# orange-vertex/depthmapX

Hardware: AMD Instinct MI355X
Metric: grid cells/sec for VISPREP makeGraph + VGA global on N×N grid (higher is better)
Workload: dtype f64

## Files before the change

### depthmapx_amd/csrc/api/vga_global.hip

```cpp

static void prep_range(const dmx_graph* g, int64_t& b, int64_t& e) {
    b = 0; e = g->nnodes;
    if (g->prep_fn && g->prep_e >= 0) { b = g->prep_b; e = g->prep_e; }
}
static int prep_allreduce(dmx_graph* g, void* p, int64_t count, int dtype) {
    if (!g->prep_fn || count <= 0) return DMX_OK;
    HIPCHK(hipStreamSynchronize(g->ctx->stream));
    if (g->prep_fn(p, count, dtype, g->prep_user) != 0)
        return fail(DMX_ERR_STATE, "prep all-reduce callback failed");
    return DMX_OK;
}
static int prepare_symmetry(dmx_graph* g);
static int build_scan_order(dmx_graph* g);
static int prepare_uf(dmx_graph* g) {
    if (g->scan_ready) return DMX_OK;
    if (int rc = prepare_symmetry(g)) return rc;
    dmx_ctx* ctx = g->ctx;
    hipStream_t s = ctx->stream;
    PointMapHost& h = *g->pm->host;
    const int cols = h.cols(), rows = h.rows();
    const int tw = (cols + 7) / 8, th = (rows + 7) / 8;
    const int64_t C = (int64_t)cols * rows, N = g->nnodes;
    DevBuf<int> cov;
    DevBuf<unsigned long long> cnt;
// ... 47 lines not shown
    if (N) {
        HIPCHK(hipMemcpyAsync(d_ss.p, ss.data(), N * 8, hipMemcpyHostToDevice, s));
        hipLaunchKernelGGL(scan_pool_kernel, dim3((unsigned)std::min<int64_t>(N, 8192)), dim3(256), 0, s, rows,
                           g->pm->d_node_cell.p, N, g->node_run_start.p, g->node_nruns.p, g->bin_nruns.p, g->pool.p, d_ss.p,
                           g->scan_pool.p, g->cell_scan_start.p, g->cell_nruns.p);
        HIPCHK(hipGetLastError());
    }
    HIPCHK(hipStreamSynchronize(s));
    g->scan_released = false;
    return DMX_OK;
}

static int restore_scan_order(dmx_graph* g) {
    if (!g->scan_released) return DMX_OK;
    g->pmask.reset(); g->ppre.reset(); g->poff.reset();
    g->tvis.reset(); g->ftvis.reset(); g->tvsum.reset(); g->tvnz.reset(); g->ttvis.reset();
    g->tvw = 0;
    g->tiles_ready = false;
    return build_scan_order(g);
}

static int prepare_symmetry(dmx_graph* g) {
    if (g->symmetric >= 0) return DMX_OK;
    const char* force = getenv("DMX_VGA_KERNEL");
    if (force && std::string(force) == "topdown") {
        g->symmetric = 0;
        g->sym_diff.reset(); g->sym_ho.reset(); g->sym_fused = false;
        return DMX_OK;
    }
    dmx_ctx* ctx = g->ctx;
    hipStream_t s = ctx->stream;
// ... 185 lines not shown
    }
    return DMX_OK;
}

static void prep_state_stats(dmx_ctx* ctx, const dmx_graph* g) {
    long long f = 0;
    if (g->scan_pool.p) f |= 1;
    if (g->scan_released) f |= 2;
    if (g->tvis.p) f |= 4;
    if (g->ftvis.p) f |= 8;
    if (g->ttvis.p) f |= 16;
    if (g->pmask.p) f |= 32;
    if (g->tvsum.p || g->tvnz.p) f |= 64;
    ctx->last_stats[40] = f;
    ctx->last_stats[41] = (long long)((g->tvis.p ? g->tvis.n * 8 : 0) + (g->ftvis.p ? g->ftvis.n * 8 : 0) +
                                      (g->ttvis.p ? g->ttvis.n * 8 : 0) + (g->tvsum.p ? g->tvsum.n * 8 : 0) + (g->tvnz.p ? g->tvnz.n * 8 : 0));
    ctx->last_stats[42] = (long long)(g->scan_pool.p ? g->scan_pool.n * sizeof(Run) : 0);
}

static size_t tile_lds_layout(int tw, int th, bool* fg, bool* rbm) {
    const size_t nt = (size_t)tw * th, wr_ = (tw + 63) / 64, wc_ = (th + 63) / 64;
    const size_t lds_f = nt * 8, lds_h = (size_t)VGA_HMAX * 4;
    const size_t lds_sc = (size_t)(th * wr_ + tw * wc_) * 8, lds_rbcb = (size_t)(th * wr_ + th * 8 * wr_ + tw * 8 * wc_) * 8;
    const size_t lds_cap = (size_t)160 * 1024 - 1024;
    const char* rb_env = getenv("DMX_VGA_RB");
    const bool rb_ok = !(rb_env && atoi(rb_env) == 0);
    *fg = false;
    *rbm = false;
    if (rb_ok && lds_f + lds_rbcb + lds_h <= lds_cap) { *rbm = true; return lds_f + lds_rbcb + lds_h; }
    if (lds_f + lds_sc + lds_h <= lds_cap) return lds_f + lds_sc + lds_h;
    if (rb_ok && lds_rbcb + lds_h <= lds_cap) { *fg = true; *rbm = true; return lds_rbcb + lds_h; }
// ... 98 lines not shown
        }
        const char* pm_env = getenv("DMX_VGA_PMASK");
        if (ftv && !(pm_env && atoi(pm_env) == 0) && (!wide || ((tvw + 63) / 64 <= 64 && nt <= 65535)))
            if (int rc = prepare_pmask(g, rows, tw, th, tvw, Ct, wide)) return rc;
        if (wide && (tvw + 63) / 64 <= 64) {
            HIPCHK(g->tvsum.alloc((size_t)Ct * ((tvw + 63) / 64)));
            hipLaunchKernelGGL(tile_vsum_kernel, dim3((unsigned)((Ct + 3) / 4)), dim3(256), 0, s, Ct, tvw, g->tvis.p,
                               g->tvsum.p);
            HIPCHK(hipGetLastError());
        }
        const char* nz_env = getenv("DMX_VGA_TVNZ");
        if (VGA_TVNZ && !wide && ftv && g->pmask.p && !(nz_env && atoi(nz_env) == 0)) {
            HIPCHK(g->tvnz.alloc((size_t)Ct * ((tvw + 63) / 64)));
            hipLaunchKernelGGL(tile_vsum_kernel, dim3((unsigned)((Ct + 3) / 4)), dim3(256), 0, s, Ct, tvw, g->tvis.p,
                               g->tvnz.p);
            HIPCHK(hipGetLastError());
        }
        g->tvw = tvw;
    }
    HIPCHK(hipStreamSynchronize(s));
    g->tiles_ready = true;
    return DMX_OK;
}

#ifndef VGA_NT_BIG
#define VGA_NT_BIG 1024
#endif
static int ordered_search(dmx_ctx* ctx, dmx_graph* g, double radius, const std::vector<int32_t>& src,
                          const std::vector<int32_t>& seed_cells, float* outp, int64_t* d_levels, int32_t* d_cell_level) {
    const PointMapHost& h = *g->pm->host;
// ... 74 lines not shown
    return rc;
}

extern "C++" template <int NT, bool SPECIAL, bool RBM, bool FG>
static int launch_tile(dmx_ctx* ctx, const VgaTileParams& Q, int64_t nsrc, size_t lds, int64_t* blocks_out,
                       DevBuf<unsigned long long>& xg, DevBuf<int4>& queue, DevBuf<int32_t>& list) {
    {
        const int64_t nt = (int64_t)Q.tw * Q.th;
        const char* why = nullptr;
        if (Q.tw != (Q.cols + 7) / 8 || Q.th != (Q.rows + 7) / 8 || nt <= 0) why = "tile grid does not cover the cells";
        else if (lds > (size_t)160 * 1024) why = "dynamic LDS above 160 KiB";
        else if (!FG && (size_t)nt * 8 > lds) why = "frontier bitmap larger than the dynamic LDS";
        else if (Q.tvis && Q.tvw != Q.th * ((Q.tw + 63) / 64)) why = "tile-visibility row width differs from the tile grid";
        else if (!FG && Q.pmask && Q.tvw > 256) why = "row words past the fused phase-C test (256)";
        else if (Q.tvnz && (FG || Q.tvw > 256)) why = "narrow row summaries on a wide grid";
        else if (Q.pmask && !FG && nt > 32767) why = "narrow mask hint: tile index above 15 bits";
        else if (Q.asym_tiles && Q.alist_cap <= 0) why = "asymmetric mode without an A-cell list";
        if (why) return fail(DMX_ERR_STATE, (std::string("VGA tile launch: ") + why).c_str());
        hipFuncAttributes fa;
        HIPCHK(hipFuncGetAttributes(&fa, reinterpret_cast<const void*>(&vga_tile_kernel<NT, SPECIAL, RBM, FG>)));
        if (fa.sharedSizeBytes + lds > (size_t)160 * 1024)
            return fail(DMX_ERR_STATE, "VGA tile launch: static plus dynamic LDS above 160 KiB");
    }
    int occ = 0;
    HIPCHK(hipOccupancyMaxActiveBlocksPerMultiprocessor(&occ, vga_tile_kernel<NT, SPECIAL, RBM, FG>, NT, lds));
    if (occ < 1) occ = 1;
    const int64_t blocks = std::max<int64_t>(1, std::min<int64_t>((int64_t)ctx->num_cu * occ, nsrc));
    const int64_t nt = (int64_t)Q.tw * Q.th;
    HIPCHK(xg.alloc((size_t)blocks * (FG ? 3 : 2) * nt));
    HIPCHK(queue.alloc((size_t)blocks * nt * 2));
// ... 28 lines not shown
    P.list = list.p;
    P.tlist = tlist.p;
    P.hint = hint.p;
    DevBuf<unsigned long long> hintw;
    P.hintw = nullptr;
    if (P.pmask && P.tvsum) {
        HIPCHK(hintw.alloc((size_t)nt * 64));
        HIPCHK(hipMemsetAsync(hintw.p, 0, (size_t)nt * 64 * 8, ctx->stream));
        P.hintw = hintw.p;
    }
    P.chunk = std::max(1, policy::hook_int("DMX_VGA_CHUNK", policy::kVgaSourceChunk));
    P.nwork = (int)((P.src_end - P.src_begin + P.chunk - 1) / P.chunk);
    P.bsplit = policy::hook_int("DMX_VGA_BSPLIT", policy::kVgaTileBSplit) & 3;
    P.csplit = policy::hook_int("DMX_VGA_CSPLIT", policy::kVgaTileCSplit) & 1;
    P.walk = policy::hook_int("DMX_VGA_WALK", policy::kVgaTileWalk) != 0;
    HIPCHK(hipEventRecord(ctx->ev0, ctx->stream));
    P.ctl = ctx->d_ctl;
    ctx->h_ctl->progress = 0;
    DevBuf<VgaTileParams> dP;
    HIPCHK(dP.alloc(1));
    HIPCHK(hipMemcpyAsync(dP.p, &P, sizeof(P), hipMemcpyHostToDevice, ctx->stream));
    hipLaunchKernelGGL((vga_tile_kernel<NT, SPECIAL, RBM, FG>), dim3((unsigned)blocks), dim3(NT), lds, ctx->stream,
                       (const VgaTileParams*)dP.p);
    HIPCHK(hipGetLastError());
    HIPCHK(wait_progress(ctx, DMX_PHASE_VGA, nsrc, P.chunk));
    *blocks_out = blocks;
    return DMX_OK;
}

static int vga_tile_impl(dmx_ctx* ctx, dmx_graph* g, double radius, int gates_only, int64_t sb, int64_t se, float* out,
// ... 12 lines not shown
        HIPCHK(d_out.alloc(std::max<int64_t>(N, 1) * 7));
        outp = d_out.p;
    }
    DevBuf<int64_t> d_lv;
    if (levels) HIPCHK(d_lv.alloc(std::max<int64_t>(N, 1) * 3));
    HIPCHK(hipMemsetAsync(ctx->counters.p, 0, 16 * sizeof(int), ctx->stream));
    HIPCHK(hipMemsetAsync(ctx->stats.p, 0, 32 * sizeof(unsigned long long), ctx->stream));
    VgaTileParams Q;
    Q.cols = h.cols(); Q.rows = h.rows(); Q.tw = tw; Q.th = th;
    Q.seed_tiles = g->notuf_tiles.p; Q.regular_tiles = g->regular_tiles.p; Q.nonexp_tiles = g->pm->d_nonexp_tiles.p;
    Q.cr = g->cr.p; Q.heads = g->heads.p; Q.tscan_start = g->tscan_start.p; Q.tnruns = g->tnruns.p;
    Q.scan_pool = g->scan_released ? g->pool.p : g->scan_pool.p;
    Q.tvis = g->tvw ? g->tvis.p : nullptr; Q.tvw = g->tvw;
    Q.tvsum = (g->tvw && g->tvsum.p) ? g->tvsum.p : nullptr;
    Q.tvnz = (g->tvw && g->tvnz.p) ? g->tvnz.p : nullptr;
    Q.ftvis = (g->tvw && g->ftvis.p) ? g->ftvis.p : nullptr;
    Q.ttvis = (g->tvw && g->ttvis.p) ? g->ttvis.p : nullptr;
    Q.ttany = Q.ttvis ? g->ttvis.p + (size_t)tw * th * g->tvw : nullptr;
    const char* pmk_env = getenv("DMX_VGA_PMASK");
    Q.pmask = (Q.ftvis && g->pmask.p && (g->scan_released || !(pmk_env && atoi(pmk_env) == 0))) ? g->pmask.p : nullptr;
    Q.poff = Q.pmask ? g->poff.p : nullptr;
    Q.ppre = Q.pmask ? g->ppre.p : nullptr;
    Q.node_cell = g->pm->d_node_cell.p; Q.cell_node = g->pm->d_cell_node.p; Q.node_flags = g->pm->d_node_flags.p;
    Q.node_run_start = g->node_run_start.p; Q.node_nruns = g->node_nruns.p; Q.pool = g->pool.p;
    const bool corr = g->nspecial > 0;
    Q.spec_index = corr ? g->spec_index.p : nullptr;
    Q.extra_off = corr ? g->extra_off.p : nullptr;
    Q.extra = corr ? g->extra.p : nullptr;
    Q.missing_off = corr ? g->missing_off.p : nullptr;
    Q.missing = corr ? g->missing.p : nullptr;
// ... 24 lines not shown
        Q.alist_cap = (int)std::max<int64_t>(pg->nasym, 1);
    }
    Q.alpha = policy::hook_int("DMX_VGA_ALPHA", policy::kVgaTileAlpha);
    Q.bext = BEXT_DEFAULT;
    if (const char* b = getenv("DMX_VGA_BEXT")) Q.bext = std::max(0, atoi(b));
    Q.crk = std::min(CRK, std::max(0, policy::hook_int("DMX_VGA_CRK", policy::kVgaTileCommonRuns)));
    Q.work_counter = ctx->counters.p + 0; Q.error = ctx->counters.p + 1;
    DevBuf<int32_t> d_hist, d_nlev;
    HIPCHK(d_hist.alloc((size_t)std::max<int64_t>(N, 1) * VGA_HMAX));
    HIPCHK(d_nlev.alloc(std::max<int64_t>(N, 1)));
    Q.maxlev = maxlev; Q.hist_out = d_hist.p; Q.nlev_out = d_nlev.p; Q.stats = ctx->stats.p;
    bool fg = false, rbm = false;
    const size_t L = tile_lds_layout(tw, th, &fg, &rbm);
    if (!L) return fail(DMX_ERR_CAPACITY, "grid too large for the tile BFS's LDS summaries");
    if (fg && !policy::hook("DMX_VGA_ALPHA")) Q.alpha = policy::kVgaTileAlphaHbm;
    DevBuf<unsigned long long> xg;
    DevBuf<int4> queue;
    DevBuf<int32_t> list;
    int64_t blocks = 0;
    int kt = 0, ntpb = 0;
    (void)kt;
    if (nsrc > 0) {
        const bool sp = g->nspecial > 0;
        if (fg) {
            rc = sp ? (rbm ? launch_tile<1024, true, true, true>(ctx, Q, nsrc, L, &blocks, xg, queue, list)
                           : launch_tile<1024, true, false, true>(ctx, Q, nsrc, L, &blocks, xg, queue, list))
                    : (rbm ? launch_tile<1024, false, true, true>(ctx, Q, nsrc, L, &blocks, xg, queue, list)
                           : launch_tile<1024, false, false, true>(ctx, Q, nsrc, L, &blocks, xg, queue, list));
            ntpb = 1024;
        } else if (nt <= 4096) {
// ... 28 lines not shown
    int hc[2];
    HIPCHK(copy_sync(ctx->stream, hc, ctx->counters.p, sizeof(hc), hipMemcpyDeviceToHost));
    if (hc[1] & ~KERR_ORDER) return fail(DMX_ERR_CAPACITY, "VGA BFS exceeded its level capacity");
    ctx->last_stats[38] = 0;
    if ((hc[1] & KERR_ORDER) && nseeds == 0)
        if (int rc2 = vga_order_rerun(ctx, g, radius, oflag.p, outp, levels ? d_lv.p : nullptr)) return rc2;
    unsigned long long st[32];
    HIPCHK(copy_sync(ctx->stream, st, ctx->stats.p, sizeof(st), hipMemcpyDeviceToHost));
    for (int i = 0; i < 5; i++) ctx->phase_cycles[i] = (long long)st[8 + i];
    ctx->last_stats[18] = (long long)st[16];
    ctx->last_stats[19] = (long long)st[17];
    ctx->last_stats[20] = (long long)st[18];
    ctx->last_stats[21] = (long long)st[19];
    ctx->last_stats[22] = (long long)st[20];
    ctx->last_stats[27] = (long long)st[25];
    ctx->last_stats[28] = (long long)st[26];
    ctx->last_stats[29] = (long long)st[27];
    ctx->last_stats[30] = (long long)st[28];
    ctx->last_stats[31] = (long long)st[29];
    ctx->last_stats[23] = (long long)st[21];
    ctx->last_stats[24] = (VGA_ROWSTAT || VGA_CSTAT) ? (long long)st[22] : 0;
    ctx->last_stats[25] = 0;
    ctx->last_stats[48] = (long long)st[23];
    ctx->last_stats[49] = (VGA_ROWSTAT || VGA_CSTAT) ? 0 : (long long)st[22];
    ctx->last_stats[26] = (long long)st[24];
    ctx->last_stats[3] = 3 | ((long long)g->nspecial << 8);
    ctx->last_stats[4] = (long long)st[0];
    ctx->last_stats[5] = (long long)(st[3] | (st[4] << 32));
    ctx->last_stats[6] = (long long)st[2];
    ctx->last_stats[7] = nsrc;
    ctx->last_stats[8] = (long long)st[5];
    ctx->last_stats[9] = (long long)st[6];
    ctx->last_stats[10] = 0;
    ctx->last_stats[11] = (long long)st[7];
    ctx->last_stats[12] = blocks | ((long long)kt << 32) | ((long long)ntpb << 40) | ((long long)fg << 56) |
                          ((long long)rbm << 57);
    ctx->last_stats[13] = (long long)st[13];
    ctx->last_stats[14] = (long long)st[14] * g->tvw * 8;
    ctx->last_stats[15] = (long long)st[15];
    ctx->last_stats[16] = (long long)st[1];
    ctx->last_stats[17] = (long long)st[14];
    ctx->last_stats[35] = (long long)st[30];
    ctx->last_stats[36] = (long long)st[31];
    ctx->last_stats[37] = (long long)(g->pmask.p ? g->pmask.n * 8 : 0);
    prep_state_stats(ctx, g);
    if (pg) {
        ctx->last_stats[40] |= 128;
        ctx->last_stats[43] = pg->nasym;
    }
    if (nseeds > 0) return DMX_OK;
    if (!out_on_device && nsrc > 0)
        HIPCHK(copy_sync(ctx->stream, out + sb * 7, d_out.p + sb * 7, nsrc * 7 * 4, hipMemcpyDeviceToHost));
    if (levels && nsrc > 0)
// ... 104 lines not shown
    if (!ctx || !g || !out) return fail(DMX_ERR_ARG, "bad arguments");
    if (g->node_begin != 0 || g->node_end != g->nnodes)
        return fail(DMX_ERR_STATE, "VGA needs the whole graph (assemble the shards first)");
    HIPCHK(hipSetDevice(ctx->device));
    const int64_t N = g->nnodes;
    if (se < 0 || se > N) se = N;
    if (sb < 0 || sb > se) return fail(DMX_ERR_ARG, "bad source range");
    int rc = prepare_uf(g);
    if (rc) return rc;
    rc = prepare_symmetry(g);
    if (rc) return rc;
    ctx->last_stats[40] = 0;
    ctx->last_stats[43] = 0;
    ctx->last_stats[48] = 0;
    ctx->last_stats[49] = 0;
    PointMapHost& h = *g->pm->host;
    const int tw = (h.cols() + 7) / 8, th = (h.rows() + 7) / 8;
    const int maxlev = 4096;
    {
        const char* fk = getenv("DMX_VGA_KERNEL");
        const bool forced_other = fk && (std::string(fk) == "v1" || std::string(fk) == "do" || std::string(fk) == "topdown");
        const int nt = tw * th;
        const bool force_asym = getenv("DMX_VGA_ASYM") && g->has_drawing && g->symmetric == 1 && g->nspecial > 0;
        if (!forced_other && g->symmetric == 1 && !ctx->tile_disabled && !force_asym) {
            int rc2 = vga_tile_impl(ctx, g, radius, gates_only, sb, se, out, out_on_device, levels, tw, th);
            if (rc2 != DMX_ERR_CAPACITY) return rc2;
        } else if (!forced_other && (g->symmetric == 0 || force_asym) && !ctx->tile_disabled && !getenv("DMX_VGA_NOASYM") &&
                   prepare_asym(ctx, g) == DMX_OK) {
            int rc2 = vga_tile_impl(ctx, g->aref.get(), radius, gates_only, sb, se, out, out_on_device, levels, tw, th,
                                    nullptr, 0, nullptr, nullptr, g);
// ... 172 lines not shown
```

### depthmapx_amd/csrc/dmx_api.hip

```cpp
#include <hip/hip_runtime.h>

#include <execinfo.h>
#include <signal.h>
#include <unistd.h>

#include <algorithm>
#include <array>
#include <chrono>
#include <cstdio>
#include <cstring>
#include <map>
#include <memory>
#include <mutex>
#include <string>
#include <thread>
#include <vector>

#include "../../include/dmx.h"
#include "policy.hpp"
#include "host/bsptree.hpp"
#include "host/graphfile.hpp"
#include "host/graphio.hpp"
#include "host/pointmap.hpp"
#include "kernels/makegraph.hip"
// ... 147 lines not shown
    int device = 0;
    bool tile_disabled = false;
    hipStream_t stream = nullptr;
    hipStream_t codec_stream = nullptr;
    hipEvent_t ev0 = nullptr, ev1 = nullptr;
    int num_cu = 0;
    double last_mk_s = 0, last_vga_s = 0, last_sd_s = 0;
    long long last_sd_stats[3] = {0, 0, 0};
    int last_sd_attempts = 0;
    long long last_sd_extra[2] = {0, 0};
    int last_sd_mode = 0;
    long long last_sd_batched[5] = {0, 0, 0, 0, 0};
    long long phase_cycles[5] = {0, 0, 0, 0, 0};
    DevBuf<int> counters;
    DevBuf<unsigned long long> stats;
    long long last_stats[50] = {};
    std::vector<int64_t> last_mk_reruns;
    DmxCtl* h_ctl = nullptr;
    DmxCtl* d_ctl = nullptr;
    dmx_progress_fn progress = nullptr;
    void* progress_user = nullptr;
    double progress_interval = 0.5;
    hipEvent_t ev_poll = nullptr;
    double last_fill_s[2] = {0, 0};
    double last_iso_bsp_s = 0, last_iso_kernel_s = 0;
    long long last_iso[4] = {0, 0, 0, 0};
    double sqrt_err = 0.0;
    long long sqrt_err_nmax = 0;
    long long last_fill_levels = 0;
    double last_conn_s[2] = {0, 0};
    long long last_conn[4] = {0, 0, 0, 0};
// ... 49 lines not shown
    int symmetric = -1;
    int nspecial = 0;
    std::vector<int32_t> special_nodes;
    DevBuf<int32_t> spec_index, extra_off, extra, missing_off, missing;
    DevBuf<unsigned long long> sym_prefix, sym_diff, sym_ho;
    bool sym_fused = false;
    bool tiles_ready = false;
    DevBuf<int64_t> tscan_start;
    DevBuf<int32_t> tnruns;
    DevBuf<Run> heads, cr;
    DevBuf<unsigned long long> tvis;
    DevBuf<unsigned long long> ftvis;
    DevBuf<unsigned long long> ttvis;
    DevBuf<unsigned long long> tvsum;
    DevBuf<unsigned long long> tvnz;
    DevBuf<unsigned long long> pmask;
    DevBuf<int64_t> poff;
    DevBuf<uint16_t> ppre;
    int tvw = 0;
    DevBuf<unsigned long long> regular_tiles;
    int64_t prep_b = 0, prep_e = -1;
    dmx_allreduce_fn prep_fn = nullptr;
    void* prep_user = nullptr;
    std::vector<double> drawing;
    bool has_drawing = false;
    int asym_state = 0;
    std::string asym_why;
    std::unique_ptr<dmx_pointmap> aref_pm;
    std::unique_ptr<dmx_graph> aref;
    DevBuf<unsigned long long> asym_tiles;
// ... 354 lines not shown
    (void)hipSetDevice(c->device);
    c->counters.reset();
    c->stats.reset();
    if (c->ev0) (void)hipEventDestroy(c->ev0);
    if (c->ev1) (void)hipEventDestroy(c->ev1);
    if (c->ev_poll) (void)hipEventDestroy(c->ev_poll);
    if (c->h_ctl) (void)hipHostFree(c->h_ctl);
    if (c->codec_stream) (void)hipStreamDestroy(c->codec_stream);
    if (c->stream) (void)hipStreamDestroy(c->stream);
    delete c;
    return DMX_OK;
}

int dmx_ctx_last_stats(dmx_ctx* c, int64_t* out, int n) {
    if (!c || !out) return fail(DMX_ERR_ARG, "bad arguments");
    for (int i = 0; i < n && i < 50; i++) out[i] = c->last_stats[i];
    return DMX_OK;
}

int dmx_ctx_last_timing(dmx_ctx* c, double* mk, double* vga) {
    if (!c) return fail(DMX_ERR_ARG, "ctx is NULL");
    if (mk) *mk = c->last_mk_s;
    if (vga) *vga = c->last_vga_s;
    return DMX_OK;
}

#include "api/pointmap.hip"
#include "api/makegraph.hip"
#include "api/shard.hip"
#include "api/vga_global.hip"
#include "api/vga_other.hip"
// ... 11 lines not shown
```

### depthmapx_amd/csrc/kernels/vga_tile.hip

```cpp
#include "common.hpp"

namespace dmx {

constexpr int KH = 8;
constexpr int CRK = 4;
constexpr int BEXT_DEFAULT = 0;
constexpr int VGA_HMAX = 64;

struct VgaTileParams {
    int cols, rows, tw, th;
    const unsigned long long* seed_tiles;
    const unsigned long long* regular_tiles;
    const unsigned long long* nonexp_tiles;
    const Run* cr;
    const Run* heads;
    const int64_t* tscan_start;
    const int32_t* tnruns;
    const Run* scan_pool;
    const unsigned long long* tvis;
    const unsigned long long* ftvis;
    const unsigned long long* ttvis;
    const unsigned long long* ttany;
    const unsigned long long* pmask;
    const int64_t* poff;
    const uint16_t* ppre;
    int tvw;
    const unsigned long long* tvsum;
    const unsigned long long* tvnz;
    const int32_t* node_cell;
    const int32_t* cell_node;
    const uint8_t* node_flags;
    const int64_t* node_run_start;
    const int32_t* node_nruns;
    const Run* pool;
    const int32_t* spec_index;
    const int32_t* extra_off;
    const int32_t* extra;
    const int32_t* missing_off;
    const int32_t* missing;
    int64_t src_begin, src_end;
    int radius, gates_only;
    int64_t uf_count;
    int alpha;
// ... 7 lines not shown
    unsigned long long* xg;
    unsigned long long* fg;
    int4* queue;
    int32_t* list;
    int32_t* tlist;
    int maxlev;
    const int32_t* seeds;
    int nseeds;
    const int32_t* src_list;
    int32_t* cell_level;
    int bext;
    int crk;
    int bsplit;
    int csplit;
    int walk;
    const int2* mpairs;
    int nmp;
    const int2* mamb;
    int nmamb;
    int32_t* mseen;
    uint8_t* oflag;
    int32_t* hist_out;
    int32_t* nlev_out;
    int* error;
    const unsigned long long* asym_tiles;
    const unsigned long long* asym_uf;
    const Run* apool;
    const int64_t* arun_start;
    const int32_t* anruns;
    int32_t* alist;
// ... 205 lines not shown
        return line_hits_rb(V.F, V.CB + x * V.wc, x >> 3, V.tw, ru.y0 >> 3, ru.y1 >> 3,
                            colm & (~0ull << (8 * (ru.y0 & 7))), colm & (~0ull >> (8 * (7 - (ru.y1 & 7)))));
    }
    if (ru.y0 == ru.y1) {
        const int y = ru.y0, ty = y >> 3;
        return line_hits<false>(V.F, V.Fsr + ty * V.wr, ty * V.tw, 1, ru.x0 >> 3, ru.x1 >> 3, ru.x0 & 7, ru.x1 & 7,
                                (y & 7) * 8);
    } else if (ru.x0 == ru.x1) {
        const int x = ru.x0, tx = x >> 3;
        return line_hits<true>(V.F, V.Fsc + tx * V.wc, tx, V.tw, ru.y0 >> 3, ru.y1 >> 3, ru.y0 & 7, ru.y1 & 7, x & 7);
    } else {
        return diag_hits(V, ru);
    }
}

struct TileShared {
    int src, qn, hn, item, bn;
    int q2n, b2n;
    int en, eitem;
    int an, aitem;
    int tn[2];
    int mpart;
    unsigned long long cnt, mass;
    unsigned long long mcorr, mdisc;
    long long m_f, m_u, disc, target;
};

__device__ __forceinline__ int grab_work(DmxCtl* ctl, int* work_counter) {
    return ctl_poll(ctl, atomicAdd(work_counter, 1));
}

__device__ __forceinline__ int run_count_f(const unsigned long long* F, int tw, Run ru) {
    int c = 0;
    if (ru.y0 == ru.y1) {
        const int y = ru.y0, ty = y >> 3, sh = (y & 7) * 8;
        for (int tx = ru.x0 >> 3; tx <= (ru.x1 >> 3); tx++) {
            const int lo = max((int)ru.x0, tx * 8) & 7, hi = min((int)ru.x1, tx * 8 + 7) & 7;
            c += __popcll(F[ty * tw + tx] & ((unsigned long long)((0xFFu >> (7 - hi)) & (0xFFu << lo) & 0xFFu) << sh));
        }
    } else if (ru.x0 == ru.x1) {
// ... 170 lines not shown
__device__ __forceinline__ unsigned long long buf_load64(__amdgpu_buffer_rsrc_t rs, int off) {
    const auto v = __builtin_amdgcn_raw_buffer_load_b64(rs, off, 0, 0);
    return (unsigned long long)v[0] | ((unsigned long long)v[1] << 32);
}
__device__ __forceinline__ void crow_load(const VgaTileParams& P, const unsigned long long* Fsr, int id, unsigned nzb,
                                          CRow& r) {
    const int lane = lanes_below(~0ull);
    const int tvw = P.tvw;
    const size_t row = (size_t)id * tvw;
    const __amdgpu_buffer_rsrc_t rt = __builtin_amdgcn_make_buffer_rsrc((void*)uni_ptr(P.tvis + row), 0, tvw * 8, 0x00020000);
    const __amdgpu_buffer_rsrc_t rf = __builtin_amdgcn_make_buffer_rsrc((void*)uni_ptr(P.ftvis + row), 0, tvw * 8, 0x00020000);
#pragma unroll
    for (int k = 0; k < 4; k++) {
        const int w = k * 64 + lane;
        const unsigned long long fs = Fsr[min(w, tvw - 1)];
        const int off = (w < tvw && fs != 0ull && ((nzb >> k) & 1u)) ? w * 8 : tvw * 8;
        r.t[k] = buf_load64(rt, off);
        r.f[k] = buf_load64(rf, off);
    }
}

__device__ __forceinline__ bool pmask_hit_rows(const VgaTileParams& P, const unsigned long long* F,
                                               const unsigned long long* Fsr, int id, unsigned& nload, uint32_t& hnew,
                                               int& how, const CRow& r, unsigned nzb = 0xFu, unsigned* rstat = nullptr) {
    const int lane = lanes_below(~0ull);
    const int tvw = P.tvw, tw = P.tw, wr = (P.tw + 63) / 64;
    const size_t row = (size_t)id * tvw;
    unsigned long long pw[4], cw[4];
    int base[4];
    bool cert = false;
    int ct = -1;
// ... 12 lines not shown
        if (rstat) {
            rstat[0] += __popcll(__ballot(fs != 0ull && ((nzb >> k) & 1u)));
            rstat[1] += __popcll(__ballot(fs != 0ull && t == 0ull));
            rstat[2] += __popcll(__ballot(fs != 0ull && f == 0ull));
        }
#endif
    }
    if (const unsigned long long cb = __ballot(cert)) {
        const int fl = __ffsll((long long)cb) - 1, ctl = __builtin_amdgcn_readlane(ct, fl);
        const int w = (ctl >> 6) * 64 + fl;
        const int t = (w / wr) * tw + (w % wr) * 64 + (ctl & 63);
        hnew = 0x80000000u | ((uint32_t)t << 16) | 0xFFFFu;
        how = 1;
        return true;
    }
    if (__ballot((cw[0] | cw[1] | cw[2] | cw[3]) != 0ull) == 0ull) { how = 2; return false; }
    how = 0;
#if VGA_PHASEC_ROWSONLY
    return false;
#endif
#if VGA_CSTAT
    if (rstat) {
        rstat[0] += __popcll(__ballot((cw[0] != 0ull))) + __popcll(__ballot((cw[1] != 0ull))) +
                    __popcll(__ballot((cw[2] != 0ull))) + __popcll(__ballot((cw[3] != 0ull)));
        unsigned pc = __popcll(cw[0]) + __popcll(cw[1]) + __popcll(cw[2]) + __popcll(cw[3]);
        for (int off = 32; off >= 1; off >>= 1) pc += __shfl_xor(pc, off);
        rstat[1] += pc;
    }
#endif
#pragma unroll
    for (int k = 0; k < 4; k++) base[k] = cw[k] ? (int)P.ppre[row + k * 64 + lane] : 0;
    const unsigned long long* pm = P.pmask + P.poff[id];
#pragma unroll 1
    for (int k = 0; k < 4; k++) {
        const int w = k * 64 + lane;
        const int trow = (w / wr) * tw + (w % wr) * 64;
        unsigned long long c = cw[k];
        const unsigned long long p = pw[k];
        const int bk = base[k];
        while (__ballot(c != 0ull) != 0ull) {
            constexpr int NM = 4;
            unsigned long long mk[NM];
            int tl[NM], sl[NM];
#if VGA_CSTAT
            if (rstat) rstat[2]++;
#endif
#pragma unroll
            for (int j = 0; j < NM; j++) {
                tl[j] = -1;
                if (c) {
                    const int b = __ffsll((long long)c) - 1;
                    c &= c - 1;
                    tl[j] = trow + b;
                    sl[j] = bk + __popcll(p & ((1ull << b) - 1ull));
                    mk[j] = pm[sl[j]];
                    nload++;
                }
            }
            int hj = -1, ht = 0, hq = 0;
// ... 794 lines not shown
                if (tid == 0) { const unsigned long long n = __builtin_amdgcn_s_memtime(); ST(10, n - tmark); tmark = n; }
                const int hn = uni(S.hn);
#if VGA_CSTAT
                if (tid == 0) atomicMax(&SC[22], (unsigned long long)hn);
#endif
                constexpr int CCH = VGA_CCH;
                constexpr int CSTEP = 4;
                const unsigned long long c_t0 = __builtin_amdgcn_s_memtime();
                for (;;) {
                    int it0 = 0;
                    if (lane == 0) it0 = atomicAdd(&S.item, CCH);
                    it0 = __builtin_amdgcn_readlane(it0, 0);
                    if (it0 >= hn) break;
                    const int cn = min(CCH, hn - it0);
                    const int myv = lane < cn ? L[it0 + lane] : -1;
                    static_assert(!VGA_TVNZ || CCH * 4 <= 64, "tvnz prefetch: 4 summary words an entry");
                    unsigned long long nzp = ~0ull;
                    if (VGA_TVNZ && !FG && P.tvnz) {
                        const int jj = lane >> 2, kk = lane & 3, tvsw = (P.tvw + 63) >> 6;
                        const int vj = __shfl(myv, jj);
                        if (jj < cn && kk < tvsw) nzp = P.tvnz[(size_t)(vj < 0 ? -1 - vj : vj) * tvsw + kk];
                    }
                    unsigned long long certain_m = 0ull, pruned_m = 0ull;
                    if (P.tvis && (!P.pmask || (FG && VGA_WIDE_ROWPASS && P.tvsum))) {
                        for (int j = 0; j < cn; j += 2) {
                            const int v0 = __builtin_amdgcn_readlane(myv, j);
                            const int v1 = __builtin_amdgcn_readlane(myv, j + 1);
                            const bool r0 = v0 >= 0, r1 = j + 1 < cn && v1 >= 0;
                            const unsigned long long* tv0 = P.tvis + (size_t)(r0 ? v0 : 0) * P.tvw;
                            const unsigned long long* tv1 = P.tvis + (size_t)(r1 ? v1 : 0) * P.tvw;
                            const unsigned long long* fv0 = P.ftvis ? P.ftvis + (size_t)(r0 ? v0 : 0) * P.tvw : nullptr;
                            const unsigned long long* fv1 = P.ftvis ? P.ftvis + (size_t)(r1 ? v1 : 0) * P.tvw : nullptr;
                            unsigned long long fa0 = 0ull, ta0 = 0ull, fa1 = 0ull, ta1 = 0ull;
                            if (!P.tvsum) {
#pragma unroll 4
                                for (int k = 0; k * 64 < P.tvw; k++) {
                                    const int w = k * 64 + lane;
                                    const unsigned long long fs = w < P.tvw ? Fsr[w] : 0ull;
// ... 48 lines not shown
                        }
                        const unsigned long long regm = __ballot(lane < cn && myv >= 0);
                        if (lane == 0) {
                            ST(14, __popcll(regm));
                            ST(16, __popcll(certain_m));
                            ST(1, __popcll(certain_m));
                            ST(13, __popcll(pruned_m));
                        }
                    }
                    unsigned long long found_m = certain_m;
                    int cf_n = 0, cf_cert = 0, cf_prun = 0, cf_hit = 0;
                    int c1n = 0;
                    const bool use_nz = VGA_TVNZ && !FG && P.tvnz;
                    const bool c1 = !VGA_PHASEC_OFF && !FG && (P.csplit & 1) && P.pmask;
                    const unsigned long long stm = c1 ? __ballot(lane < cn && myv >= 0) & ~(certain_m | pruned_m) : 0ull;
                    if (stm) {
                        const C1Out co = c1_chunk(P, F, Fsr, Hn, SC, myv, stm, nzp, use_nz);
                        found_m |= co.found;
                        nlt += co.nl;
                        cf_n += __popcll(stm);
                        cf_cert += co.cert;
                        cf_prun += co.prun;
                        cf_hit += __popcll(co.found);
                        c1n = __popcll(stm);
                    }
                    for (int j = 0; j < cn; j++) {
                        if (((certain_m | pruned_m | stm) >> j) & 1ull) continue;
                        int id = __builtin_amdgcn_readlane(myv, j);
                        const bool special = id < 0;
                        if (special) id = -1 - id;
                        bool found = false;
                        int nr = 0;
                        const unsigned nzb = chunk_nzb(nzp, j, use_nz);
                        if (SPECIAL && special) {
                            int x, y;
                            xy_of_tile_id(id, tw, x, y);
                            int nmiss = 1;
                            if (P.pmask) found = special_extra_hit(P, F, P.cell_node[x * rows + y], &nmiss);
                            if (!found && nmiss == 0) {
// ... 64 lines not shown
                        else if (lane == 0) ST(6, nr);
                    }
                    if (lane < cn && ((found_m >> lane) & 1ull)) {
                        const int id = myv < 0 ? -1 - myv : myv;
                        or_wg(&Xg[id >> 6], 1ull << (id & 63));
                    }
                    if (lane == 0) ST(5, cn - __popcll(found_m));
                    if (lane == 0 && cf_n) {
                        ST(14, cf_n);
                        ST(31, cf_n);
                        if (cf_cert) ST(16, cf_cert);
                        if (cf_prun) ST(13, cf_prun);
                        if (cf_hit) ST(1, cf_hit);
#if !VGA_ROWSTAT && !VGA_CSTAT
                        if (c1n) ST(22, c1n);
#endif
                    }
                }
                if (lane == 0) ST(21, __builtin_amdgcn_s_memtime() - c_t0);
            } else {
                for (int t = tid; t < nt; t += NT) {
                    unsigned long long f = F[t];
                    const int c = __popcll(f);
                    int pos = c ? atomicAdd(&S.hn, c) : 0;
                    while (f) {
                        const int b = __ffsll((long long)f) - 1;
                        f &= f - 1;
                        L[pos++] = (t << 6) | b;
                    }
                }
// ... 61 lines not shown
                }
                __syncthreads();
                if (tid == 0) { S.an = 0; S.aitem = 0; }
                __syncthreads();
            }
            {
                const unsigned long long n = __builtin_amdgcn_s_memtime();
                if (tid == 0) {
                    if (bottom_up) ST(11, n - tmark);
                    else ST(level == 0 ? 8 : 17, n - tmark);
                }
                tmark = n;
            }
            const bool have_list = level > 0;
            for (int i = tid; i < nfs; i += NT) Fsr[i] = 0ull;
            if (have_list)
                for (int t = tid; t < nt; t += NT) F[t] = 0ull;
            __syncthreads();
            unsigned long long c_loc = 0, m_loc = 0;
            const int32_t* TLc = TL + (level & 1) * nt;
            int32_t* TLn = TL + ((level + 1) & 1) * nt;
            const int nwalk = have_list ? uni(S.tn[level & 1]) : nt;
            if (tid == 0 && have_list) atomicMax(&SC[23], (unsigned long long)nwalk);
            const bool fused0 = plain && !have_list;
            const bool nonexp = P.radius != -1 || seeded;
            if (walk)
            for (int i0 = 0; i0 < nwalk; i0 += WNF * NT) {
                int tt[WNF];
                if (have_list) {
#pragma unroll
// ... 151 lines not shown
                        const int n = min(64, th - w * 64);
                        for (int j = 0; j < n; j++) {
                            unsigned long long y = F[(w * 64 + j) * tw + tx];
                            y |= y >> 32;
                            y |= y >> 16;
                            y |= y >> 8;
#pragma unroll
                            for (int k = 0; k < 8; k++) b[k] |= ((y >> k) & 1ull) << j;
                        }
#pragma unroll
                        for (int k = 0; k < 8; k++) CB[(tx * 8 + k) * wc + w] = b[k];
                    }
                }
            }
            sync_global();
            const long long cnt = uni64(S.cnt), mass = uni64(S.mass);
            const long long mcorr = uni64(S.mcorr), mdisc = uni64(S.mdisc);
            if (tid == 0) { const unsigned long long n = __builtin_amdgcn_s_memtime(); ST(12, n - tmark); tmark = n; }
            __syncthreads();
            if (tid == 0) {
                S.cnt = 0; S.mass = 0; S.qn = 0; S.hn = 0; S.item = 0; S.bn = 0; S.mcorr = 0; S.mdisc = 0;
                S.q2n = 0; S.b2n = 0; S.en = 0; S.eitem = 0;
                S.tn[level & 1] = 0;
                S.disc += cnt + mdisc;
                S.m_u -= cnt + mdisc;
                S.m_f = mass;
            }
            __syncthreads();
            if (cnt == 0) break;
            if (level + 1 >= VGA_HMAX) { overflow = true; break; }
// ... 284 lines not shown
}

__global__ void tile_vsum_kernel(int64_t Ct, int tvw, const unsigned long long* tvis, unsigned long long* tvsum) {
    const int lane = threadIdx.x & 63;
    const int64_t c = (int64_t)blockIdx.x * (blockDim.x >> 6) + (threadIdx.x >> 6);
    if (c >= Ct) return;
    const int tvsw = (tvw + 63) / 64;
    const unsigned long long* row = tvis + (size_t)c * tvw;
    for (int j = 0; j < tvsw; j++) {
        const int w = j * 64 + lane;
        const unsigned long long bits = __ballot(w < tvw && row[w] != 0ull);
        if (lane == 0) tvsum[(size_t)c * tvsw + j] = bits;
    }
}

struct LSeg {
    int x0, y0, dx, dy, len;
};
__device__ __forceinline__ LSeg lseg_of(Run ru) {
    LSeg s;
    s.x0 = ru.x0;
    s.y0 = ru.y0;
    if (ru.y0 == ru.y1) { s.dx = 1; s.dy = 0; s.len = ru.x1 - ru.x0 + 1; }
    else if (ru.x0 == ru.x1) { s.dx = 0; s.dy = 1; s.len = ru.y1 - ru.y0 + 1; }
    else { s.dx = 1; s.dy = (ru.y1 > ru.y0) ? 1 : -1; s.len = ru.x1 - ru.x0 + 1; }
    return s;
}
__device__ __forceinline__ void lseg_overlap(const LSeg& c, const LSeg& s, int* pa, int* pb) {
    *pa = 1;
    *pb = 0;
// ... 152 lines not shown
```

### depthmapx_amd/csrc/policy.hpp

```cpp
#pragma once
#include <cstdint>
#include <cstdlib>

namespace dmx {
namespace policy {

constexpr int64_t kMkSample = 4096;
constexpr double kMkSourceCost = 0.0, kMkChunkCost = 0.7;

constexpr int kVgaTileAlpha = 60;
constexpr int kVgaTileAlphaHbm = 1000;
constexpr int kVgaTileCommonRuns = 4;
constexpr int kVgaSourceChunk = 1;
constexpr int kVgaTileBSplit = 3;
constexpr int kVgaTileCSplit = 1;
constexpr int kVgaTileWalk = 1;
constexpr int kVgaDoAlpha = 15;
constexpr int kVgaDoShortList = 16;

constexpr int kSdbAmbCap = 1 << 16;
constexpr int kSdbEntCap = 1 << 22;

constexpr int kTvWindow = 64;
constexpr int kTvWindowMaxBytes = 64 * 1024;

constexpr int kIsoGapCap = 32;
constexpr int kIsoBlockCap = 128;
constexpr int kIsoRetryFactor = 16;
constexpr int kIsoCapMax = 1 << 16;
constexpr int kIsoWavesPerCu = 8;
// ... 23 lines not shown
```

### depthmapx_amd/engine.py

```python
import ctypes
import math

import numpy as np

from . import _native as N

MAKEGRAPH_COLUMNS = ["Connectivity", "Point First Moment", "Point Second Moment"]
STEPDEPTH_COLUMNS = ["Metric Step Shortest-Path Angle", "Metric Step Shortest-Path Length",
                     "Metric Straight-Line Distance"]
VGA_LOCAL_COLUMNS = ["Visual Clustering Coefficient", "Visual Control", "Visual Controllability"]
VGA_METRIC_COLUMNS = ["Metric Mean Shortest-Path Angle", "Metric Mean Shortest-Path Distance",
                      "Metric Mean Straight-Line Distance", "Metric Node Count"]
VGA_ANGULAR_COLUMNS = ["Angular Mean Depth", "Angular Total Depth", "Angular Node Count"]
VGA_COLUMNS = ["Visual Entropy", "Visual Integration [HH]", "Visual Integration [P-value]",
               "Visual Integration [Tekl]", "Visual Mean Depth", "Visual Node Count",
               "Visual Relativised Entropy"]


def isovist_cone(angle, viewangle, degrees=False):
    angle, viewangle = float(angle), float(viewangle)
    if degrees:
        angle = angle / 180.0 * math.pi
        viewangle = viewangle / 180.0 * math.pi
    if viewangle >= 2 * math.pi:
# ... 139 lines not shown
        n = ctypes.c_int64()
        N.check(N.lib().dmx_ctx_last_mk_reruns(self.h, None, 0, ctypes.byref(n)))
        out = np.zeros(max(n.value, 1), dtype=np.int64)
        N.check(N.lib().dmx_ctx_last_mk_reruns(self.h, N.ptr(out), n.value, ctypes.byref(n)))
        out = out[:n.value]
        cap = (out >> 62) & 1
        nodes = out & ((1 << 62) - 1)
        return np.unique(nodes[cap == 0]), np.unique(nodes[cap == 1])

    def last_phase_cycles(self):
        out = np.zeros(5, dtype=np.int64)
        N.check(N.lib().dmx_ctx_last_phase_cycles(self.h, N.ptr(out)))
        return dict(zip(["level1", "tile_common", "heads", "hard", "bookkeeping"], (int(v) for v in out)))

    def last_stats(self):
        out = np.zeros(50, dtype=np.int64)
        N.check(N.lib().dmx_ctx_last_stats(self.h, N.ptr(out), 50))
        keys = ["mk_cells_examined", "mk_visible_pairs", "mk_runs", "vga_kernel", "vga_runs_expanded", "vga_levels",
                "vga_cells_reached", "vga_sources", "vga_fail_cells", "vga_fail_runs", "vga_hbm_bitmaps",
                "vga_cr_tiles", "vga_launch", "vga_pruned_cells", "vga_tvis_bytes", "vga_hard_runs", "vga_hard_hits",
                "vga_hard_cells", "vga_hard_certain", "vga_topdown_cycles", "vga_b_tiles", "vga_b_cells", "vga_tt_tiles", "vga_c_busy", "vga_c_scan", "vga_c_spec", "vga_n_spec", "vga_tt_pruned", "vga_b_row_cycles", "vga_b_cell_tiles",
                "vga_b_cell_cycles", "vga_b_ext_cells", "mk_depth_steps", "mk_chunks", "mk_reruns", "vga_pmask_loads", "vga_pmask_cells", "vga_pmask_bytes",
                "vga_order_reruns", "vga_sym_scatter_us", "vga_prep_flags", "vga_tile_rows_bytes", "vga_scan_bytes",
                "vga_asym_nodes", "tv_lines", "tv_pixel_steps", "tv_window", "mk_diag_inexact", "vga_tl_max", "vga_c_row_cells"]
        d = {k: int(v) for k, v in zip(keys, out)}
        lv = d.pop("vga_levels")
        d["vga_bottom_up_levels"], d["vga_top_down_levels"] = lv & 0xFFFFFFFF, lv >> 32
        d["vga_special_nodes"] = d["vga_kernel"] >> 8
        d["vga_frontier_hbm"] = (d["vga_launch"] >> 56) & 1
        d["vga_line_summaries"] = (d["vga_launch"] >> 57) & 1
        d["vga_threads"] = (d["vga_launch"] >> 40) & 0xFFFF
        d["vga_launch"] &= (1 << 32) - 1
        f = d["vga_prep_flags"]
        d["vga_scan_order"], d["vga_scan_released"] = f & 1, (f >> 1) & 1
        d["vga_prep"] = "+".join(n for b, n in enumerate(["scan", "scan-released", "tvis", "ftvis", "ttvis", "masks",
                                                            "tvsum", "asymmetric-mode"]) if (f >> b) & 1) or "none"
        d["vga_asym_mode"] = (f >> 7) & 1
        d["vga_kernel"] = ["topdown-v1", "direction-optimizing(top-down only)",
                           "direction-optimizing", "tile-resolved"][d["vga_kernel"] & 0xFF]
# ... 358 lines not shown
```

Measured before the change: 178,300.

## Prune phase-C cells with coarse 8x8 tile-block visibility summaries

Precomputes, per cell, a 256-bit summary of which 8x8 tile blocks it can see, and maintains a matching block-level summary of the current frontier in shared memory each level. In phase C, cells whose block summary does not meet the frontier are marked as pruned before the finer c1_chunk row test runs, which avoids the per-row loads for those cells. It adds a prep kernel, extra global memory, atomics per level and a new stats slot. It is gated to narrow grids with 256 or fewer blocks.

Result: faster. 184,000, median of 6 (+3.2%).

```diff
diff --git a/depthmapx_amd/csrc/api/vga_global.hip b/depthmapx_amd/csrc/api/vga_global.hip
--- a/depthmapx_amd/csrc/api/vga_global.hip
+++ b/depthmapx_amd/csrc/api/vga_global.hip
@@ -85,7 +85,7 @@
 static int restore_scan_order(dmx_graph* g) {
     if (!g->scan_released) return DMX_OK;
     g->pmask.reset(); g->ppre.reset(); g->poff.reset();
-    g->tvis.reset(); g->ftvis.reset(); g->tvsum.reset(); g->tvnz.reset(); g->ttvis.reset();
+    g->tvis.reset(); g->ftvis.reset(); g->tvsum.reset(); g->tvnz.reset(); g->tvblk.reset(); g->ttvis.reset();
     g->tvw = 0;
     g->tiles_ready = false;
     return build_scan_order(g);
@@ -301,7 +301,8 @@
     if (g->tvsum.p || g->tvnz.p) f |= 64;
     ctx->last_stats[40] = f;
     ctx->last_stats[41] = (long long)((g->tvis.p ? g->tvis.n * 8 : 0) + (g->ftvis.p ? g->ftvis.n * 8 : 0) +
-                                      (g->ttvis.p ? g->ttvis.n * 8 : 0) + (g->tvsum.p ? g->tvsum.n * 8 : 0) + (g->tvnz.p ? g->tvnz.n * 8 : 0));
+                                      (g->ttvis.p ? g->ttvis.n * 8 : 0) + (g->tvsum.p ? g->tvsum.n * 8 : 0) + (g->tvnz.p ? g->tvnz.n * 8 : 0) +
+                                      (g->tvblk.p ? g->tvblk.n * 8 : 0));
     ctx->last_stats[42] = (long long)(g->scan_pool.p ? g->scan_pool.n * sizeof(Run) : 0);
 }
 
@@ -430,6 +431,12 @@
             HIPCHK(g->tvnz.alloc((size_t)Ct * ((tvw + 63) / 64)));
             hipLaunchKernelGGL(tile_vsum_kernel, dim3((unsigned)((Ct + 3) / 4)), dim3(256), 0, s, Ct, tvw, g->tvis.p,
                                g->tvnz.p);
+            HIPCHK(hipGetLastError());
+        }
+        if (!wide && ftv && g->pmask.p && ((tw + 7) / 8) * ((th + 7) / 8) <= 256) {
+            HIPCHK(g->tvblk.alloc((size_t)Ct * 4));
+            hipLaunchKernelGGL(tile_vblk_kernel, dim3((unsigned)((Ct + 3) / 4)), dim3(256), 0, s, Ct, tvw, (tw + 63) / 64,
+                               (tw + 7) / 8, g->tvis.p, g->tvblk.p);
             HIPCHK(hipGetLastError());
         }
         g->tvw = tvw;
@@ -534,6 +541,7 @@
         else if (Q.tvis && Q.tvw != Q.th * ((Q.tw + 63) / 64)) why = "tile-visibility row width differs from the tile grid";
         else if (!FG && Q.pmask && Q.tvw > 256) why = "row words past the fused phase-C test (256)";
         else if (Q.tvnz && (FG || Q.tvw > 256)) why = "narrow row summaries on a wide grid";
+        else if (Q.tvblk && (FG || ((Q.tw + 7) / 8) * ((Q.th + 7) / 8) > 256)) why = "tile-block summaries past 256 blocks";
         else if (Q.pmask && !FG && nt > 32767) why = "narrow mask hint: tile index above 15 bits";
         else if (Q.asym_tiles && Q.alist_cap <= 0) why = "asymmetric mode without an A-cell list";
         if (why) return fail(DMX_ERR_STATE, (std::string("VGA tile launch: ") + why).c_str());
@@ -592,6 +600,7 @@
     P.bsplit = policy::hook_int("DMX_VGA_BSPLIT", policy::kVgaTileBSplit) & 3;
     P.csplit = policy::hook_int("DMX_VGA_CSPLIT", policy::kVgaTileCSplit) & 1;
     P.walk = policy::hook_int("DMX_VGA_WALK", policy::kVgaTileWalk) != 0;
+    P.ccert = policy::hook_int("DMX_VGA_CCERT", policy::kVgaTileCCert) != 0;
     HIPCHK(hipEventRecord(ctx->ev0, ctx->stream));
     P.ctl = ctx->d_ctl;
     ctx->h_ctl->progress = 0;
@@ -634,6 +643,7 @@
     Q.tvis = g->tvw ? g->tvis.p : nullptr; Q.tvw = g->tvw;
     Q.tvsum = (g->tvw && g->tvsum.p) ? g->tvsum.p : nullptr;
     Q.tvnz = (g->tvw && g->tvnz.p) ? g->tvnz.p : nullptr;
+    Q.tvblk = (g->tvw && g->tvblk.p) ? g->tvblk.p : nullptr;
     Q.ftvis = (g->tvw && g->ftvis.p) ? g->ftvis.p : nullptr;
     Q.ttvis = (g->tvw && g->ttvis.p) ? g->ttvis.p : nullptr;
     Q.ttany = Q.ttvis ? g->ttvis.p + (size_t)tw * th * g->tvw : nullptr;
@@ -688,6 +698,7 @@
     const size_t L = tile_lds_layout(tw, th, &fg, &rbm);
     if (!L) return fail(DMX_ERR_CAPACITY, "grid too large for the tile BFS's LDS summaries");
     if (fg && !policy::hook("DMX_VGA_ALPHA")) Q.alpha = policy::kVgaTileAlphaHbm;
+    if (fg) Q.tvblk = nullptr;
     DevBuf<unsigned long long> xg;
     DevBuf<int4> queue;
     DevBuf<int32_t> list;
@@ -746,7 +757,7 @@
     ctx->last_stats[21] = (long long)st[19];
     ctx->last_stats[22] = (long long)st[20];
     ctx->last_stats[27] = (long long)st[25];
-    ctx->last_stats[28] = (long long)st[26];
+    ctx->last_stats[28] = (VGA_ROWSTAT || VGA_CSTAT) ? (long long)st[26] : 0;
     ctx->last_stats[29] = (long long)st[27];
     ctx->last_stats[30] = (long long)st[28];
     ctx->last_stats[31] = (long long)st[29];
@@ -755,6 +766,8 @@
     ctx->last_stats[25] = 0;
     ctx->last_stats[48] = (long long)st[23];
     ctx->last_stats[49] = (VGA_ROWSTAT || VGA_CSTAT) ? 0 : (long long)st[22];
+    const long long ncert = (VGA_ROWSTAT || VGA_CSTAT) ? 0 : (long long)st[26];
+    ctx->last_stats[50] = ncert;
     ctx->last_stats[26] = (long long)st[24];
     ctx->last_stats[3] = 3 | ((long long)g->nspecial << 8);
     ctx->last_stats[4] = (long long)st[0];
@@ -768,7 +781,7 @@
     ctx->last_stats[12] = blocks | ((long long)kt << 32) | ((long long)ntpb << 40) | ((long long)fg << 56) |
                           ((long long)rbm << 57);
     ctx->last_stats[13] = (long long)st[13];
-    ctx->last_stats[14] = (long long)st[14] * g->tvw * 8;
+    ctx->last_stats[14] = ((long long)st[14] - ncert) * g->tvw * 8;
     ctx->last_stats[15] = (long long)st[15];
     ctx->last_stats[16] = (long long)st[1];
     ctx->last_stats[17] = (long long)st[14];
@@ -903,6 +916,7 @@
     ctx->last_stats[43] = 0;
     ctx->last_stats[48] = 0;
     ctx->last_stats[49] = 0;
+    ctx->last_stats[50] = 0;
     PointMapHost& h = *g->pm->host;
     const int tw = (h.cols() + 7) / 8, th = (h.rows() + 7) / 8;
     const int maxlev = 4096;
diff --git a/depthmapx_amd/csrc/dmx_api.hip b/depthmapx_amd/csrc/dmx_api.hip
--- a/depthmapx_amd/csrc/dmx_api.hip
+++ b/depthmapx_amd/csrc/dmx_api.hip
@@ -185,7 +185,7 @@
     long long phase_cycles[5] = {0, 0, 0, 0, 0};
     DevBuf<int> counters;
     DevBuf<unsigned long long> stats;
-    long long last_stats[50] = {};
+    long long last_stats[51] = {};
     std::vector<int64_t> last_mk_reruns;
     DmxCtl* h_ctl = nullptr;
     DmxCtl* d_ctl = nullptr;
@@ -265,6 +265,7 @@
     DevBuf<unsigned long long> ttvis;
     DevBuf<unsigned long long> tvsum;
     DevBuf<unsigned long long> tvnz;
+    DevBuf<unsigned long long> tvblk;
     DevBuf<unsigned long long> pmask;
     DevBuf<int64_t> poff;
     DevBuf<uint16_t> ppre;
@@ -649,7 +650,7 @@
 
 int dmx_ctx_last_stats(dmx_ctx* c, int64_t* out, int n) {
     if (!c || !out) return fail(DMX_ERR_ARG, "bad arguments");
-    for (int i = 0; i < n && i < 50; i++) out[i] = c->last_stats[i];
+    for (int i = 0; i < n && i < 51; i++) out[i] = c->last_stats[i];
     return DMX_OK;
 }
 
diff --git a/depthmapx_amd/csrc/kernels/vga_tile.hip b/depthmapx_amd/csrc/kernels/vga_tile.hip
--- a/depthmapx_amd/csrc/kernels/vga_tile.hip
+++ b/depthmapx_amd/csrc/kernels/vga_tile.hip
@@ -27,6 +27,7 @@
     int tvw;
     const unsigned long long* tvsum;
     const unsigned long long* tvnz;
+    const unsigned long long* tvblk;
     const int32_t* node_cell;
     const int32_t* cell_node;
     const uint8_t* node_flags;
@@ -64,6 +65,7 @@
     int bsplit;
     int csplit;
     int walk;
+    int ccert;
     const int2* mpairs;
     int nmp;
     const int2* mamb;
@@ -299,6 +301,17 @@
     }
 }
 
+__device__ __forceinline__ void blk_place(unsigned long long t, int w, int wr, int nbc, int& wd, unsigned long long& lo,
+                                          unsigned long long& hi) {
+    unsigned v = 0u;
+#pragma unroll
+    for (int i = 0; i < 8; i++) v |= (unsigned)(((t >> (8 * i)) & 0xFFull) != 0ull) << i;
+    const int p = ((w / wr) >> 3) * nbc + (w % wr) * 8, sh = p & 63;
+    wd = p >> 6;
+    lo = (unsigned long long)v << sh;
+    hi = sh > 56 ? (unsigned long long)v >> (64 - sh) : 0ull;
+}
+
 struct TileShared {
     int src, qn, hn, item, bn;
     int q2n, b2n;
@@ -309,6 +322,7 @@
     unsigned long long cnt, mass;
     unsigned long long mcorr, mdisc;
     long long m_f, m_u, disc, target;
+    unsigned long long fblk[4];
 };
 
 __device__ __forceinline__ int grab_work(DmxCtl* ctl, int* work_counter) {
@@ -509,7 +523,11 @@
     for (int k = 0; k < 4; k++) {
         const int w = k * 64 + lane;
         const unsigned long long fs = Fsr[min(w, tvw - 1)];
+#if VGA_CSTAT == 2
+        const int off = w < tvw ? w * 8 : tvw * 8;
+#else
         const int off = (w < tvw && fs != 0ull && ((nzb >> k) & 1u)) ? w * 8 : tvw * 8;
+#endif
         r.t[k] = buf_load64(rt, off);
         r.f[k] = buf_load64(rf, off);
     }
@@ -552,12 +570,41 @@
         how = 1;
         return true;
     }
-    if (__ballot((cw[0] | cw[1] | cw[2] | cw[3]) != 0ull) == 0ull) { how = 2; return false; }
+    if (__ballot((cw[0] | cw[1] | cw[2] | cw[3]) != 0ull) == 0ull) {
+#if VGA_CSTAT == 2
+        if (rstat) {
+            bool ma = false, mb = false;
+#pragma unroll
+            for (int k = 0; k < 4; k++) {
+                const int w = k * 64 + lane;
+                const unsigned long long fs = w < tvw ? Fsr[min(w, tvw - 1)] : 0ull;
+                ma |= r.t[k] != 0ull && fs != 0ull;
+                unsigned cb = 0u, fb = 0u;
+#pragma unroll
+                for (int i = 0; i < 8; i++) {
+                    cb |= (unsigned)(((r.t[k] >> (8 * i)) & 0xFFull) != 0ull) << i;
+                    fb |= (unsigned)(((fs >> (8 * i)) & 0xFFull) != 0ull) << i;
+                }
+#pragma unroll
+                for (int sft = 2; sft <= 8; sft <<= 1) {
+                    cb |= __shfl_xor(cb, sft);
+                    fb |= __shfl_xor(fb, sft);
+                }
+                mb |= (cb & fb) != 0u;
+            }
+            rstat[0] += 1u;
+            rstat[1] += __ballot(ma) == 0ull;
+            rstat[2] += wr == 2 && __ballot(mb) == 0ull;
+        }
+#endif
+        how = 2;
+        return false;
+    }
     how = 0;
 #if VGA_PHASEC_ROWSONLY
     return false;
 #endif
-#if VGA_CSTAT
+#if VGA_CSTAT == 1
     if (rstat) {
         rstat[0] += __popcll(__ballot((cw[0] != 0ull))) + __popcll(__ballot((cw[1] != 0ull))) +
                     __popcll(__ballot((cw[2] != 0ull))) + __popcll(__ballot((cw[3] != 0ull)));
@@ -580,7 +627,7 @@
             constexpr int NM = 4;
             unsigned long long mk[NM];
             int tl[NM], sl[NM];
-#if VGA_CSTAT
+#if VGA_CSTAT == 1
             if (rstat) rstat[2]++;
 #endif
 #pragma unroll
@@ -1405,7 +1452,7 @@
                     if (it0 >= hn) break;
                     const int cn = min(CCH, hn - it0);
                     const int myv = lane < cn ? L[it0 + lane] : -1;
-                    static_assert(!VGA_TVNZ || CCH * 4 <= 64, "tvnz prefetch: 4 summary words an entry");
+                    static_assert(CCH * 4 <= 64, "summary prefetch: 4 words an entry");
                     unsigned long long nzp = ~0ull;
                     if (VGA_TVNZ && !FG && P.tvnz) {
                         const int jj = lane >> 2, kk = lane & 3, tvsw = (P.tvw + 63) >> 6;
@@ -1413,6 +1460,17 @@
                         if (jj < cn && kk < tvsw) nzp = P.tvnz[(size_t)(vj < 0 ? -1 - vj : vj) * tvsw + kk];
                     }
                     unsigned long long certain_m = 0ull, pruned_m = 0ull;
+                    int ncert = 0;
+                    if (!VGA_PHASEC_OFF && !FG && P.ccert && P.tvblk && P.pmask) {
+                        const int ln = lanes_below(~0ull);
+                        const int jj = ln >> 2, kk = ln & 3;
+                        const int vj = __shfl(myv, jj);
+                        unsigned long long cb = 0ull;
+                        if (jj < cn && vj >= 0) cb = P.tvblk[(size_t)vj * 4 + kk];
+                        const unsigned long long meet = __ballot((cb & S.fblk[kk]) != 0ull);
+                        pruned_m = __ballot(ln < cn && myv >= 0 && ((meet >> (4 * (ln & 15))) & 0xFull) == 0ull);
+                        ncert = __popcll(pruned_m);
+                    }
                     if (P.tvis && (!P.pmask || (FG && VGA_WIDE_ROWPASS && P.tvsum))) {
                         for (int j = 0; j < cn; j += 2) {
                             const int v0 = __builtin_amdgcn_readlane(myv, j);
@@ -1491,6 +1549,11 @@
                     const bool use_nz = VGA_TVNZ && !FG && P.tvnz;
                     const bool c1 = !VGA_PHASEC_OFF && !FG && (P.csplit & 1) && P.pmask;
                     const unsigned long long stm = c1 ? __ballot(lane < cn && myv >= 0) & ~(certain_m | pruned_m) : 0ull;
+                    if (ncert) {
+                        cf_n += ncert;
+                        cf_prun += ncert;
+                        if (c1) c1n += ncert;
+                    }
                     if (stm) {
                         const C1Out co = c1_chunk(P, F, Fsr, Hn, SC, myv, stm, nzp, use_nz);
                         found_m |= co.found;
@@ -1499,7 +1562,7 @@
                         cf_cert += co.cert;
                         cf_prun += co.prun;
                         cf_hit += __popcll(co.found);
-                        c1n = __popcll(stm);
+                        c1n += __popcll(stm);
                     }
                     for (int j = 0; j < cn; j++) {
                         if (((certain_m | pruned_m | stm) >> j) & 1ull) continue;
@@ -1594,6 +1657,7 @@
                         if (cf_hit) ST(1, cf_hit);
 #if !VGA_ROWSTAT && !VGA_CSTAT
                         if (c1n) ST(22, c1n);
+                        if (ncert) ST(26, ncert);
 #endif
                     }
                 }
@@ -1685,6 +1749,7 @@
             }
             const bool have_list = level > 0;
             for (int i = tid; i < nfs; i += NT) Fsr[i] = 0ull;
+            if (tid < 4) S.fblk[tid] = 0ull;
             if (have_list)
                 for (int t = tid; t < nt; t += NT) F[t] = 0ull;
             __syncthreads();
@@ -1866,6 +1931,16 @@
                 }
             }
             sync_global();
+            if (!FG && P.tvblk && tid < P.th * wr) {
+                const unsigned long long fw = Fsr[tid];
+                if (fw) {
+                    int wd;
+                    unsigned long long lo, hi;
+                    blk_place(fw, tid, wr, (tw + 7) >> 3, wd, lo, hi);
+                    atomicOr(&S.fblk[wd], lo);
+                    if (hi) atomicOr(&S.fblk[min(wd + 1, 3)], hi);
+                }
+            }
             const long long cnt = uni64(S.cnt), mass = uni64(S.mass);
             const long long mcorr = uni64(S.mcorr), mdisc = uni64(S.mdisc);
             if (tid == 0) { const unsigned long long n = __builtin_amdgcn_s_memtime(); ST(12, n - tmark); tmark = n; }
@@ -2180,6 +2255,32 @@
     }
 }
 
+__global__ void tile_vblk_kernel(int64_t Ct, int tvw, int wr, int nbc, const unsigned long long* tvis, unsigned long long* tvblk) {
+    const int lane = threadIdx.x & 63;
+    const int64_t c = (int64_t)blockIdx.x * (blockDim.x >> 6) + (threadIdx.x >> 6);
+    if (c >= Ct) return;
+    const unsigned long long* row = tvis + (size_t)c * tvw;
+    unsigned long long a0 = 0ull, a1 = 0ull, a2 = 0ull, a3 = 0ull;
+    for (int w = lane; w < tvw; w += 64) {
+        const unsigned long long t = row[w];
+        if (t == 0ull) continue;
+        int wd;
+        unsigned long long lo, hi;
+        blk_place(t, w, wr, nbc, wd, lo, hi);
+        a0 |= wd == 0 ? lo : 0ull;
+        a1 |= wd == 1 ? lo : (wd == 0 ? hi : 0ull);
+        a2 |= wd == 2 ? lo : (wd == 1 ? hi : 0ull);
+        a3 |= wd == 3 ? lo : (wd == 2 ? hi : 0ull);
+    }
+    for (int off = 32; off >= 1; off >>= 1) {
+        a0 |= __shfl_xor(a0, off);
+        a1 |= __shfl_xor(a1, off);
+        a2 |= __shfl_xor(a2, off);
+        a3 |= __shfl_xor(a3, off);
+    }
+    if (lane < 4) tvblk[(size_t)c * 4 + lane] = lane == 0 ? a0 : lane == 1 ? a1 : lane == 2 ? a2 : a3;
+}
+
 struct LSeg {
     int x0, y0, dx, dy, len;
 };
diff --git a/depthmapx_amd/csrc/policy.hpp b/depthmapx_amd/csrc/policy.hpp
--- a/depthmapx_amd/csrc/policy.hpp
+++ b/depthmapx_amd/csrc/policy.hpp
@@ -14,6 +14,7 @@
 constexpr int kVgaSourceChunk = 1;
 constexpr int kVgaTileBSplit = 3;
 constexpr int kVgaTileCSplit = 1;
+constexpr int kVgaTileCCert = 1;
 constexpr int kVgaTileWalk = 1;
 constexpr int kVgaDoAlpha = 15;
 constexpr int kVgaDoShortList = 16;
diff --git a/depthmapx_amd/engine.py b/depthmapx_amd/engine.py
--- a/depthmapx_amd/engine.py
+++ b/depthmapx_amd/engine.py
@@ -177,15 +177,16 @@
         return dict(zip(["level1", "tile_common", "heads", "hard", "bookkeeping"], (int(v) for v in out)))
 
     def last_stats(self):
-        out = np.zeros(50, dtype=np.int64)
-        N.check(N.lib().dmx_ctx_last_stats(self.h, N.ptr(out), 50))
+        out = np.zeros(51, dtype=np.int64)
+        N.check(N.lib().dmx_ctx_last_stats(self.h, N.ptr(out), 51))
         keys = ["mk_cells_examined", "mk_visible_pairs", "mk_runs", "vga_kernel", "vga_runs_expanded", "vga_levels",
                 "vga_cells_reached", "vga_sources", "vga_fail_cells", "vga_fail_runs", "vga_hbm_bitmaps",
                 "vga_cr_tiles", "vga_launch", "vga_pruned_cells", "vga_tvis_bytes", "vga_hard_runs", "vga_hard_hits",
                 "vga_hard_cells", "vga_hard_certain", "vga_topdown_cycles", "vga_b_tiles", "vga_b_cells", "vga_tt_tiles", "vga_c_busy", "vga_c_scan", "vga_c_spec", "vga_n_spec", "vga_tt_pruned", "vga_b_row_cycles", "vga_b_cell_tiles",
                 "vga_b_cell_cycles", "vga_b_ext_cells", "mk_depth_steps", "mk_chunks", "mk_reruns", "vga_pmask_loads", "vga_pmask_cells", "vga_pmask_bytes",
                 "vga_order_reruns", "vga_sym_scatter_us", "vga_prep_flags", "vga_tile_rows_bytes", "vga_scan_bytes",
-                "vga_asym_nodes", "tv_lines", "tv_pixel_steps", "tv_window", "mk_diag_inexact", "vga_tl_max", "vga_c_row_cells"]
+                "vga_asym_nodes", "tv_lines", "tv_pixel_steps", "tv_window", "mk_diag_inexact", "vga_tl_max", "vga_c_row_cells",
+                "vga_c_cert_cells"]
         d = {k: int(v) for k, v in zip(keys, out)}
         lv = d.pop("vga_levels")
         d["vga_bottom_up_levels"], d["vga_top_down_levels"] = lv & 0xFFFFFFFF, lv >> 32
```
